# albtad01/NBody-EuroHPC

Hardware: AMD Instinct MI355X
Metric: body-interactions/s (higher is better)
Workload: dtype f32; 1 GPU; murb galaxy N=200000 steps=474 dt=3600 soft=2e8 seed=0 fp32 — BASELINE.json configs[2]: N=200000 i=200, 1 x MI355X; n_bodies=200000, parallelism=1 gpu, kernel_variant=8, jsplit=1, sym_waves=4, taper_pct=5, sym_passes=1

## Files before the change

include/murbhip.h:

```cpp
#ifndef MURBHIP_H_
#define MURBHIP_H_

#include <stddef.h>

#ifdef __cplusplus
extern "C" {
#endif

typedef struct murbhip_ctx murbhip_ctx;

#define MURBHIP_UNIQUE_ID_BYTES 128

#define MURBHIP_E_INVALID (-2000)
#define MURBHIP_E_STATE (-2001)
#define MURBHIP_E_NO_DEVICE (-2002)
#define MURBHIP_E_NO_RCCL (-2003)
#define MURBHIP_E_NOMEM (-2004)


int murbhip_version(void);

const char* murbhip_error_string(int code);

int murbhip_partition(unsigned long n, int world, int rank, unsigned long* first, unsigned long* count);

unsigned long murbhip_slice_slots(unsigned long n, int world);

unsigned long murbhip_slot_of_body(unsigned long n, int world, unsigned long i);

int murbhip_schedule_items(unsigned long n, int world, int rank, int split, int* pairs, unsigned long capacity,
                           unsigned long* count, unsigned long* own_count);

int murbhip_schedule_layout(unsigned long n, int world, int rank, int split, int waves, int taper_pct, int tri_first_pct,
                            int exchange_mode, long* items, unsigned long item_capacity, unsigned long* item_count, long* rows,
                            unsigned long row_capacity, unsigned long* row_count, unsigned long* floats_main,
                            unsigned long* floats_tri);


int murbhip_device_count(int* count);

int murbhip_create(murbhip_ctx** out, unsigned long n, float soft, float g, int device);

int murbhip_create_sharded(murbhip_ctx** out, unsigned long n, float soft, float g, int ndev, const int* devices,
                           int exchange);

int murbhip_unique_id(void* id_out );
int murbhip_create_rank(murbhip_ctx** out, unsigned long n, float soft, float g, int device, int rank, int world,
                        const void* unique_id);

int murbhip_destroy(murbhip_ctx* ctx);


int murbhip_upload(murbhip_ctx* ctx, const float* qx, const float* qy, const float* qz, const float* vx,
                   const float* vy, const float* vz, const float* m);

int murbhip_init_bodies(murbhip_ctx* ctx, const char* scheme, unsigned long seed);

int murbhip_download_mass(murbhip_ctx* ctx, float* m, float* r);

int murbhip_download_state(murbhip_ctx* ctx, float* qx, float* qy, float* qz, float* vx, float* vy, float* vz);

int murbhip_download_acc(murbhip_ctx* ctx, float* ax, float* ay, float* az);


int murbhip_compute_acc(murbhip_ctx* ctx);

int murbhip_compute_acc_jerk(murbhip_ctx* ctx);

int murbhip_download_jerk(murbhip_ctx* ctx, float* jx, float* jy, float* jz);
// ... 44 lines not shown
```

nbody-eurohpc_amd/csrc/murb_choose.h:

```cpp
#ifndef MURB_CHOOSE_H_
#define MURB_CHOOSE_H_

#include <algorithm>
#include <cstddef>

#include "murb_layout.h"
#include "murb_plan.h"

namespace {

struct PlanInputs {
    unsigned long n = 0;
    int world = 1;
    unsigned long slice = 0;
    unsigned long slots = 0;
    int cu_count = 0;
    size_t device_mem = 0;
    int resident_per_cu = 0;
    int variant = 0, jsplit = 0;
    int sym_waves = 0;
    int taper = -1;
    int diag_tri = -1;
    int sym_red = -1;
    int fuse_integrate = 1;
    long sym_pass_mb = 0;
    int tri_div = 0;
};

constexpr int kMaxParts = 64;
constexpr int kNumVariants = 8;
constexpr int kOneSidedVariant = 1;
constexpr int kOneSidedFewBodies = 2;
constexpr int kPersistentVariant = 7;
constexpr int kSymmetricVariant = 8;
constexpr unsigned long kSymmetricMinBodies = 2049;
constexpr int kRowsPerLaunch = kMaxParts / 2;

struct Plan {
    int variant;
    int parts_local, parts_remote;
    bool persistent;
    bool symmetric;
    int split;
    int waves;
    int taper;
    bool diag_tri;
    int red;
    MurbSchedule sched[2];
};

constexpr double kSymFastMaxReach = 0x1p34;
constexpr double kSymFastMinSoft = 0x1p-40;
inline bool sym_wide_needed(double reach, double soft) { return !(reach <= kSymFastMaxReach && soft >= kSymFastMinSoft); }
inline bool sym_wide_chosen(int option, bool needed) { return option < 0 ? needed : option != 0; }

inline int resident_blocks(const PlanInputs& in) { return std::max(in.resident_per_cu, 1) * std::max(in.cu_count, 1); }

inline MurbSchedule make_schedule(const PlanInputs& in, long groups, long tiles, int row_base)
{
    MurbSchedule sc{(int)groups, (int)tiles, 1, row_base};
    const long units = groups * tiles;
    if (units <= 0) { sc.nblocks = 0; return sc; }
    const long slots = resident_blocks(in);
    long rounds = in.jsplit > 0 ? in.jsplit : std::min<long>(8, std::max<long>(1, units / (slots * 8)));
    long nb = std::min(units, slots * rounds);
    nb = std::min(nb, std::max<long>(1, (kRowsPerLaunch - 2) * groups));
    sc.nblocks = (int)std::max<long>(nb, 1);
    return sc;
}

inline int variant_group(int variant)
{
    switch (variant) {
        case kPersistentVariant: return 32;
        case kSymmetricVariant: return 32;
        case 2: case 6: return 16;
        case 5: return 64;
        default: return 32;
    }
}
// ... 33 lines not shown
{
    const unsigned long T = in.slots / MURB_SYM_BLOCK;
    return in.fuse_integrate && in.jsplit == 0 && (T <= 4 || T == 6);
}

inline Plan make_plan(const PlanInputs& in)
{
    Plan p{};
    const auto fits = [&](int split) { return in.world == 1 || in.device_mem == 0 || sym_row_bytes(in, split) < in.device_mem / 2; };
    if (in.variant >= 1 && in.variant <= kNumVariants) p.variant = in.variant;
    else if (in.world == 1) p.variant = (in.n >= kSymmetricMinBodies && !fused_one_sided_wins(in) && fits(1)) ? kSymmetricVariant : kOneSidedVariant;
    else p.variant = (sym_items_per_rank(in) >= 400 && fits(1)) ? kSymmetricVariant : (in.slice <= 16384 ? kOneSidedFewBodies : kOneSidedVariant);
    p.symmetric = p.variant == kSymmetricVariant;
    if (p.symmetric) {
        const long items = sym_items_per_rank(in);
        const long want = (in.world > 1 ? 16L : 8L) * 4 * std::max(in.cu_count, 1);
        p.split = (in.jsplit == 1 || in.jsplit == 2 || in.jsplit == 4 || in.jsplit == 8 || in.jsplit == 16)
                      ? in.jsplit
                      : (items >= want ? 1 : (2 * items >= want ? 2 : (in.world == 1 || items >= 1000 ? 4 : (items >= 400 ? 8 : 16))));
        struct SmallPlan { int waves, split, taper; bool diag_tri; };
        static const SmallPlan kSmallPlans[5] = {{8, 4, 30, true}, {4, 4, 5, false}, {4, 8, 5, false}, {8, 8, 30, true}, {4, 16, 5, false}};
        static const signed char kSmallPlanOfBlocks[25] = {4, 4, 4, 3, 3, 3, 4,
                                                           3, 3, 0, 2, 2, 1, 3, 0, 2, 1, 2, 0, 1, 2, 0, 1, 0, 2};
        const int T = (int)(in.slots / MURB_SYM_BLOCK);
        const bool small = in.world == 1 && T <= 27;
        const SmallPlan sp = kSmallPlans[(small && in.cu_count == 256 && T >= 3) ? kSmallPlanOfBlocks[T - 3] : (T < 10 ? 3 : 0)];
        p.waves = (in.sym_waves == 4 || in.sym_waves == 8) ? in.sym_waves : (small ? sp.waves : 4);
        if (in.jsplit == 0 && in.sym_waves == 0 && small) p.split = sp.split;
        while (p.split > 1 && MURB_SYM_BLOCK / p.split < 16 * p.waves) p.split /= 2;
        while (p.split > 1 && !fits(p.split)) p.split /= 2;
        p.taper = in.taper >= 0 ? in.taper : (in.world > 1 ? 0 : (small ? sp.taper : (in.n <= 600000 ? 5 : 0)));
        p.diag_tri = in.diag_tri >= 0 ? in.diag_tri != 0 : (small && sp.diag_tri);
        p.red = in.sym_red >= 0 ? in.sym_red : 1;
        p.persistent = false;
        p.parts_local = p.parts_remote = 0;
        return p;
    }
    const unsigned long tiles_local = in.slice / MURB_TILE_BODIES;
    const unsigned long tiles_remote = (in.slots - in.slice) / MURB_TILE_BODIES;
    p.persistent = p.variant == kPersistentVariant;
    if (p.persistent) {
        unsigned long first, count;
        partition(in.n, in.world, 0, &first, &count);
        const long groups = (long)((count + 31) / 32);
        p.sched[0] = make_schedule(in, groups, (long)tiles_local, 0);
        p.sched[1] = make_schedule(in, groups, (long)tiles_remote, kRowsPerLaunch);
        p.parts_local = p.parts_remote = 0;
        return p;
    }
    if (in.world == 1) {
        p.parts_local = in.jsplit > 0 ? std::min<int>(in.jsplit, (int)std::min<unsigned long>(tiles_local, kMaxParts))
                                      : auto_parts(in, p.variant, in.slice, tiles_local);
        if (in.jsplit == 0 && in.fuse_integrate && p.variant == kOneSidedVariant && in.slots / MURB_SYM_BLOCK <= 6) p.parts_local = 1;
        p.parts_remote = 0;
    } else {
        const unsigned long tiles_all = tiles_local + tiles_remote;
        int total = in.jsplit > 0 ? in.jsplit : auto_parts(in, p.variant, in.slice, tiles_all);
        total = std::max(total, 2);
        int loc = (int)std::max<unsigned long>(1ul, (unsigned long)total * tiles_local / tiles_all);
        int rem = std::max(1, total - loc);
        p.parts_local = (int)std::min<unsigned long>((unsigned long)loc, std::min<unsigned long>(tiles_local, kMaxParts / 2));
        p.parts_remote = (int)std::min<unsigned long>((unsigned long)rem, std::min<unsigned long>(tiles_remote, kMaxParts / 2));
    }
    return p;
}

inline int plan_tri_div(const PlanInputs& in, const Plan& p)
{
    if (in.tri_div > 0) return in.tri_div;
    if (in.world == 1) return 1;
    const long tb = (long)(in.slice / MURB_SYM_BLOCK);
    const long items = tb * (tb + 1) / 2 * p.split / 2;
    const long slots = 4L * std::max(in.cu_count, 1) * 4 / p.waves;
    int div = 1;
    while (div < 4 && items * div < 2 * slots && MURB_SYM_BLOCK / (p.split * div * 2) >= 16 * p.waves) div *= 2;
    return div;
}

inline SymLayoutKey sym_layout_key(const PlanInputs& in, const Plan& p, bool exchange_mode, int overlap, int tri_first_pct, bool xcd_order,
                                   bool pad_aware)
{
    SymLayoutKey k;
    k.split = p.split; k.waves = p.waves; k.taper = p.taper; k.diag_tri = p.diag_tri;
    k.exchange_mode = exchange_mode;
    k.overlap = exchange_mode ? overlap : 0;
    k.tri_first_pct = exchange_mode ? tri_first_pct : 0;
    k.xcd_order = xcd_order;
    k.budget_floats = sym_pass_budget(in) / (3 * sizeof(float));
    k.tri_div = plan_tri_div(in, p);
    k.pad_aware = pad_aware;
    return k;
}

inline int hermite_parts(const PlanInputs& in)
{
    const unsigned long tiles = in.slots / MURB_TILE_BODIES;
    if (in.jsplit > 0) return (int)std::min<unsigned long>((unsigned long)in.jsplit, std::min<unsigned long>(tiles, kMaxParts / 2));
    return auto_parts(in, kOneSidedFewBodies, in.slots, tiles);
}

}

#endif
```

nbody-eurohpc_amd/csrc/murb_plan.h:

```cpp
#ifndef MURB_PLAN_H_
#define MURB_PLAN_H_

#include <cstddef>
#include <map>
#include <utility>
#include <vector>

#include "murb_schedule.h"
#include "murb_sym_types.h"

namespace {

struct SymPass {
    int item_first = 0, item_count = 0;
    int table_first = 0, table_count = 0;
    size_t floats = 0;
};

inline std::vector<std::pair<size_t, size_t>> cut_passes(const std::vector<SymPiece>& pieces, size_t budget_floats)
{
    std::vector<std::pair<size_t, size_t>> out;
    size_t first = 0, used = 0, k = 0;
    while (k < pieces.size()) {
        size_t e = k, rows = 0;
// ... 25 lines not shown
    for (size_t k = first; k < end; ++k) {
        const SymPiece& pc = pieces[k];
        const int bi = index[pc.i_slot0 / MURB_SYM_BLOCK];
        auto f = irow[bi].find(pc.J);
        if (f == irow[bi].end()) f = irow[bi].emplace(pc.J, table[bi].ni++).first;
        item_irow[k - first] = f->second;
        item_jrow[k - first] = pc.j_side() ? table[index[pc.J]].nj++ : -1;
    }
    size_t floats = 0;
    for (MurbSymBlockRows& br : table) {
        br.base_j = floats; floats += (size_t)br.nj * MURB_SYM_BLOCK;
        br.base_i = floats; floats += (size_t)br.ni * MURB_SYM_BLOCK;
    }
    for (size_t k = first; k < end; ++k) {
        const SymPiece& pc = pieces[k];
        MurbSymItem& it = items[k];
        it.i_slot0 = pc.i_slot0;
        it.ngroups = pc.len / (waves * MURB_SYM_R);
        it.J = pc.J;
        it.flags = pc.flags;
        const MurbSymBlockRows& bi = table[index[pc.i_slot0 / MURB_SYM_BLOCK]];
        it.ioff = bi.base_i + (size_t)item_irow[k - first] * MURB_SYM_BLOCK + (size_t)(pc.i_slot0 % MURB_SYM_BLOCK);
        it.joff = pc.j_side() ? table[index[pc.J]].base_j + (size_t)item_jrow[k - first] * MURB_SYM_BLOCK : 0;
    }
    return floats;
}

struct SymHostLayout {
    std::vector<MurbSymItem> items;
    int own = 0, t1 = 0;
    std::vector<MurbSymBlockRows> table_main, table_tri;
    size_t floats_main = 0, floats_tri = 0;
    std::vector<SymPass> passes;
};

struct SymLayoutKey {
    int split = 1, waves = 4, taper = 0;
    bool diag_tri = false;
    bool exchange_mode = false;
    int overlap = 0, tri_first_pct = 0;
    bool xcd_order = false;
    size_t budget_floats = 0;
    int tri_div = 1;
    bool pad_aware = true;
    bool operator==(const SymLayoutKey& o) const
    {
        return split == o.split && waves == o.waves && taper == o.taper && diag_tri == o.diag_tri && exchange_mode == o.exchange_mode &&
               overlap == o.overlap && tri_first_pct == o.tri_first_pct && xcd_order == o.xcd_order && budget_floats == o.budget_floats &&
               tri_div == o.tri_div && pad_aware == o.pad_aware;
    }
};

inline void plan_sym_layout(int W, int r, const SymFill& fill, const SymLayoutKey& key, SymHostLayout& L)
{
    const int tb = fill.tb;
    std::vector<int> flat;
    int own = 0;
    size_t t1 = 0;
    std::vector<SymPiece> pieces;
    std::vector<size_t> piece_ends;
    const auto build_pieces = [&](bool interleaved) {
        sym_schedule_items(W, r, tb, key.split, fill, flat, &own, interleaved);
        const size_t n_all = flat.size() / 2;
        t1 = (key.exchange_mode && key.overlap == 1) ? (size_t)((long)own * key.tri_first_pct / 100) : 0;
        std::vector<size_t> launch_ends;
        std::vector<int> launch_div;
        if (key.exchange_mode) {
            if (t1 > 0) { launch_ends.push_back(t1); launch_div.push_back(key.tri_div); }
            if ((size_t)own > t1) { launch_ends.push_back((size_t)own); launch_div.push_back(key.tri_div); }
            if (n_all > (size_t)own) { launch_ends.push_back(n_all); launch_div.push_back(1); }
        } else {
            launch_ends.push_back(n_all);
        }
        sym_pieces(flat, key.split, key.taper, 16 * key.waves, key.diag_tri, fill, launch_ends, pieces, piece_ends, launch_div);
    };
    build_pieces(key.xcd_order);
    if (!key.exchange_mode && key.xcd_order && cut_passes(pieces, key.budget_floats).size() > 1) build_pieces(false);
    size_t own_pieces = pieces.size();
    if (key.exchange_mode && flat.size() / 2 > (size_t)own) own_pieces = piece_ends.size() >= 2 ? piece_ends[piece_ends.size() - 2] : 0;
    L.items.assign(pieces.size(), MurbSymItem{});
    L.table_main.clear(); L.table_tri.clear();
    L.floats_main = L.floats_tri = 0;
    if (key.exchange_mode) {
        L.floats_tri = layout_sym_set(pieces, 0, own_pieces, key.waves, L.items, L.table_tri, [&](int b) { return std::make_pair(0, b - r * tb); });
        L.floats_main = layout_sym_set(pieces, own_pieces, pieces.size(), key.waves, L.items, L.table_main,
                                       [&](int b) { return std::make_pair(b / tb, b % tb); });
        L.passes.assign(1, SymPass{(int)own_pieces, (int)(pieces.size() - own_pieces), 0, (int)L.table_main.size(), L.floats_main});
    } else {
        L.passes.clear();
        std::vector<MurbSymBlockRows> table;
        for (const auto& range : cut_passes(pieces, key.budget_floats)) {
            const size_t floats = layout_sym_set(pieces, range.first, range.second, key.waves, L.items, table, [&](int b) { return std::make_pair(0, b); });
            L.passes.push_back(SymPass{(int)range.first, (int)(range.second - range.first), (int)L.table_main.size(), (int)table.size(), floats});
            L.table_main.insert(L.table_main.end(), table.begin(), table.end());
            L.floats_main = std::max(L.floats_main, floats);
        }
    }
    L.own = (int)own_pieces;
    L.t1 = t1 > 0 ? (int)piece_ends[0] : 0;
}

}

#endif
```

nbody-eurohpc_amd/csrc/murb_schedule.h:

```cpp
#ifndef MURB_SCHEDULE_H_
#define MURB_SCHEDULE_H_

#include <algorithm>
#include <vector>

#include "murb_layout.h"

namespace {

inline void partition(unsigned long n, int world, int rank, unsigned long* first, unsigned long* count)
{
    const unsigned long base = n / (unsigned long)world, rem = n % (unsigned long)world;
    const unsigned long r = (unsigned long)rank;
    *count = base + (r < rem ? 1 : 0);
    *first = r * base + std::min(r, rem);
}

inline unsigned long slice_slots(unsigned long n, int world)
{
    unsigned long first, count;
    partition(n, world, 0, &first, &count);
    return murb_round_up_tile(std::max(count, 1ul));
}

// ... 79 lines not shown
            const size_t row_first = flat.size();
            for (int j = 0; j < tb; ++j) {
                if (shared && !((r == lo) ? (a < hb) : (j >= hb))) continue;
                int ib, jb;
                sym_orient(fill, r * tb + a, s * tb + j, &ib, &jb);
                if (ib == r * tb + a) { flat.push_back(ib); flat.push_back(jb); }
                else sym_push_block_pair(fill, split, ib, jb, swapped);
            }
            const std::vector<int> row(flat.begin() + (long)row_first, flat.end());
            flat.resize(row_first);
            const int len = MURB_SLICE_ALIGN / split, real = fill.of(r * tb + a);
            for (int q = 0; q < split && q * len < real; ++q)
                for (size_t k = 0; k < row.size(); k += 2) { flat.push_back(row[k] * split + q); flat.push_back(row[k + 1]); }
        }
        flat.insert(flat.end(), swapped.begin(), swapped.end());
    }
    if (!xcd_order) return;
    const size_t n_own = (size_t)*own, n_all = flat.size() / 2;
    if (W == 1) { xcd_interleave(flat, 0, n_all); return; }
    xcd_interleave(flat, 0, n_own / 2);
    xcd_interleave(flat, n_own / 2, n_own);
    xcd_interleave(flat, n_own, n_all);
}

struct SymPiece {
    int i_slot0, len, J, flags;
    bool diag() const { return i_slot0 / MURB_SLICE_ALIGN == J; }
    bool j_side() const { return (flags & 1) == 0; }
};
constexpr int kSymStepBodies = 128;

inline void sym_pieces(const std::vector<int>& flat, int split, int taper_pct, int min_len, bool diag_tri, const SymFill& fill,
                       const std::vector<size_t>& launch_ends, std::vector<SymPiece>& out, std::vector<size_t>& piece_launch_ends,
                       const std::vector<int>& launch_div = std::vector<int>())
{
    const int len = MURB_SLICE_ALIGN / split;
    out.clear();
    piece_launch_ends.clear();
    size_t first = 0;
    for (size_t l = 0; l < launch_ends.size(); ++l) {
        const size_t end = launch_ends[l];
        const int base_div = l < launch_div.size() ? launch_div[l] : 1;
        const double total = (double)(end - first);
        for (size_t k = first; k < end; ++k) {
            const int isub = flat[2 * k], J = flat[2 * k + 1];
            const bool diag = isub / split == J;
            const double before = (double)(k - first) / (total > 0 ? total : 1.0);
            int div = 1;
            while (div < base_div && len / (2 * div) >= min_len) div *= 2;
            if (taper_pct > 0) {
                const double left = 1.0 - before;
                for (double f = taper_pct / 100.0; left <= f && len / (2 * div) >= min_len; f *= 0.5) div *= 2;
            }
            if (diag && diag_tri)
                while (len / div > kSymStepBodies && len / (2 * div) >= min_len) div *= 2;
            const int real_end = (isub / split) * MURB_SLICE_ALIGN + fill.of(isub / split);
            for (int q = 0; q < div; ++q) {
                SymPiece pc{isub * len + q * (len / div), len / div, J, diag ? 1 : 0};
                if (pc.i_slot0 >= real_end) break;
                if (pc.i_slot0 + pc.len > real_end) pc.len = (real_end - pc.i_slot0 + min_len - 1) / min_len * min_len;
                if (diag && diag_tri && pc.len <= kSymStepBodies) {
                    const int in_block = pc.i_slot0 % MURB_SLICE_ALIGN;
                    const int a = in_block / kSymStepBodies, b = (in_block + pc.len + kSymStepBodies - 1) / kSymStepBodies;
                    pc.flags = 2 | (a << 8) | (b << 12) | (b >= MURB_SLICE_ALIGN / kSymStepBodies ? 1 : 0);
                }
                out.push_back(pc);
            }
        }
        piece_launch_ends.push_back(out.size());
        first = end;
    }
}

}

#endif
```

nbody-eurohpc_amd/csrc/murbhip.hip:

```cpp
#include <hip/hip_runtime.h>

#include <algorithm>
#include <cmath>
#include <cstdio>
#include <cstdlib>
#include <cstring>
#include <functional>
#include <new>
#include <string>
#include <type_traits>
#include <vector>

#include "../../include/murbhip.h"
#include "murb_init.h"
#include "murb_ctx.h"

namespace {

constexpr int kPotentialKernel = 100;

inline bool is_idle(const murbhip_ctx* c, const Shard& sh) { return c->solo_shard >= 0 && sh.rank != c->solo_shard; }

template <int MODE, int R, int WAVES, int STAGE>
int launch_force_t(const MurbForceArgs& a, int i_slots, hipStream_t s)
// ... 1049 lines not shown
    partition(n, world, rank, first, count);
    return 0;
}

unsigned long murbhip_slice_slots(unsigned long n, int world) { return world < 1 ? 0 : slice_slots(n, world); }

unsigned long murbhip_slot_of_body(unsigned long n, int world, unsigned long i)
{
    if (world < 1 || i >= n) return ~0ul;
    const unsigned long base = n / (unsigned long)world, rem = n % (unsigned long)world;
    unsigned long r, first;
    if (i < rem * (base + 1)) { r = i / (base + 1); first = r * (base + 1); }
    else { r = rem + (base ? (i - rem * (base + 1)) / base : 0); first = rem * (base + 1) + (r - rem) * base; }
    return r * slice_slots(n, world) + (i - first);
}

int murbhip_schedule_items(unsigned long n, int world, int rank, int split, int* pairs, unsigned long capacity,
                           unsigned long* count, unsigned long* own_count)
{
    if (world < 1 || world > MURB_SYM_MAX_RANKS || rank < 0 || rank >= world || !count || !own_count) return MURBHIP_E_INVALID;
    if (split != 1 && split != 2 && split != 4 && split != 8 && split != 16) return MURBHIP_E_INVALID;
    std::vector<int> flat;
    int own = 0;
    sym_schedule_items(world, rank, (int)(slice_slots(n, world) / MURB_SYM_BLOCK), split, sym_fill(n, world), flat, &own);
    *count = flat.size() / 2;
    *own_count = (unsigned long)own;
    if (pairs) {
        if (capacity < flat.size() / 2) return MURBHIP_E_INVALID;
        std::memcpy(pairs, flat.data(), flat.size() * sizeof(int));
    }
    return 0;
}

int murbhip_schedule_layout(unsigned long n, int world, int rank, int split, int waves, int taper_pct, int tri_first_pct,
                            int exchange_mode, long* items, unsigned long item_capacity, unsigned long* item_count, long* rows,
                            unsigned long row_capacity, unsigned long* row_count, unsigned long* floats_main,
                            unsigned long* floats_tri)
{
    if (world < 1 || world > MURB_SYM_MAX_RANKS || rank < 0 || rank >= world || !item_count || !row_count) return MURBHIP_E_INVALID;
    if (split != 1 && split != 2 && split != 4 && split != 8 && split != 16) return MURBHIP_E_INVALID;
    if ((waves != 4 && waves != 8) || taper_pct < 0 || (taper_pct & 0xff) > 100 || taper_pct > 0x7ff || tri_first_pct < 0 || tri_first_pct > 100)
        return MURBHIP_E_INVALID;
    if (MURB_SYM_BLOCK / split < 16 * waves) return MURBHIP_E_INVALID;
    SymHostLayout L;
    SymLayoutKey key;
    key.split = split; key.waves = waves; key.taper = taper_pct & 0xff; key.diag_tri = (taper_pct & 0x100) != 0;
    key.exchange_mode = exchange_mode != 0 || world > 1;
    key.overlap = 1; key.tri_first_pct = tri_first_pct; key.tri_div = 1 << ((taper_pct >> 9) & 3);
    plan_sym_layout(world, rank, sym_fill(n, world), key, L);
    *item_count = L.items.size();
    *row_count = L.table_main.size() + L.table_tri.size();
    if (floats_main) *floats_main = L.floats_main;
    if (floats_tri) *floats_tri = L.floats_tri;
    if (items) {
        if (item_capacity < L.items.size()) return MURBHIP_E_INVALID;
        const bool ex = key.exchange_mode;
        for (size_t k = 0; k < L.items.size(); ++k) {
            const MurbSymItem& it = L.items[k];
            long* o = items + 8 * k;
            o[0] = it.i_slot0; o[1] = (long)it.ngroups * waves * MURB_SYM_R; o[2] = it.J; o[3] = it.flags;
            o[4] = (ex && (int)k < L.own) ? 1 : 0;
            o[5] = (long)it.ioff; o[6] = (long)it.joff;
            o[7] = !ex ? 0 : ((int)k < L.t1 ? 0 : ((int)k < L.own ? 1 : 2));
        }
    }
    if (rows) {
        if (row_capacity < *row_count) return MURBHIP_E_INVALID;
        size_t e = 0;
        for (int set = 0; set < 2; ++set)
            for (const MurbSymBlockRows& br : (set == 0 ? L.table_main : L.table_tri)) {
                long* o = rows + 7 * e++;
                o[0] = set; o[1] = br.out_slice; o[2] = br.out_block; o[3] = (long)br.base_i; o[4] = br.ni; o[5] = (long)br.base_j; o[6] = br.nj;
            }
    }
    return 0;
}

int murbhip_device_count(int* count)
{
    if (!count) return MURBHIP_E_INVALID;
    *count = 0;
    return hip_rc(hipGetDeviceCount(count));
}

int murbhip_create(murbhip_ctx** out, unsigned long n, float soft, float g, int device)
{
    const int rank0 = 0;
    return create_common(out, n, soft, g, 1, 1, &device, &rank0, 0, false);
}

int murbhip_create_sharded(murbhip_ctx** out, unsigned long n, float soft, float g, int ndev, const int* devices,
                           int exchange)
{
    if (ndev < 1 || ndev > 64 || !devices || (exchange != 0 && exchange != 1)) return MURBHIP_E_INVALID;
    if ((unsigned long)ndev > n) return MURBHIP_E_INVALID;
    std::vector<int> ranks(ndev);
    for (int i = 0; i < ndev; ++i) ranks[i] = i;
    if (exchange == 1) {
        if (!rccl().ok) return MURBHIP_E_NO_RCCL;
    }
    RC_TRY(create_common(out, n, soft, g, ndev, ndev, devices, ranks.data(), exchange, false));
    if (exchange == 1 && ndev > 1) {
        std::vector<rccl_comm_t> comms(ndev);
        const int rc = nccl_rc(rccl().CommInitAll(comms.data(), ndev, devices));
        if (rc != 0) { murbhip_destroy(*out); *out = nullptr; return rc; }
        for (int i = 0; i < ndev; ++i) (*out)->shards[i].comm_rccl = comms[i];
    }
    return 0;
// ... 761 lines not shown
    double sums[MURB_METRIC_VALUES];
    RC_TRY(device_metrics(c, false, sums));
    std::memcpy(out10, sums + 2, 10 * sizeof(double));
    return 0;
}

int murbhip_set_option(murbhip_ctx* c, const char* key, long value)
{
    if (!c || !key) return MURBHIP_E_INVALID;
    const std::string k(key);
    if (k == "solo_shard" || k == "force_exchange") c->acc_current = false;
    if (k == "variant") { if (value < 0 || value > kNumVariants) return MURBHIP_E_INVALID; c->in.variant = (int)value; }
    else if (k == "jsplit") { if (value < 0 || value > kMaxParts / 2) return MURBHIP_E_INVALID; c->in.jsplit = (int)value; }
    else if (k == "xcd_order") c->xcd_order = value ? 1 : 0;
    else if (k == "pad_aware") c->pad_aware = value ? 1 : 0;
    else if (k == "energy_sweep") c->energy_sweep = value ? 1 : 0;
    else if (k == "sym_wide") {
        if (value < -1 || value > 1) return MURBHIP_E_INVALID;
        if ((int)value != c->sym_wide) { c->acc_current = false; c->pe_current = false; }
        c->sym_wide = (int)value;
    }
    else if (k == "fuse_integrate") c->in.fuse_integrate = value ? 1 : 0;
    else if (k == "exchange_p2p") {
        if (value && (c->exchange != 1 || !rccl().Send || !rccl().Recv)) return MURBHIP_E_STATE;
        RC_TRY(murbhip_sync(c));
        c->exchange_p2p = value ? 1 : 0;
    }
    else if (k == "tri_div") { if (value != 0 && value != 1 && value != 2 && value != 4 && value != 8) return MURBHIP_E_INVALID; c->in.tri_div = (int)value; }
    else if (k == "init_libm_fma") { if (value < -1 || value > 1) return MURBHIP_E_INVALID; c->init_libm_fma = (int)value; }
    else if (k == "tri_first_pct") { if (value < 0 || value > 100) return MURBHIP_E_INVALID; c->tri_first_pct = (int)value; }
    else if (k == "taper") { if (value < -1 || value > 100) return MURBHIP_E_INVALID; c->in.taper = (int)value; }
    else if (k == "sym_pass_mb") { if (value < 0) return MURBHIP_E_INVALID; c->in.sym_pass_mb = value; }
    else if (k == "diag_tri") { if (value < -1 || value > 1) return MURBHIP_E_INVALID; c->in.diag_tri = (int)value; }
    else if (k == "sym_red") { if (value < -1 || value > 1) return MURBHIP_E_INVALID; c->in.sym_red = (int)value; }
    else if (k == "sym_waves") { if (value != 0 && value != 4 && value != 8) return MURBHIP_E_INVALID; c->in.sym_waves = (int)value; }
    else if (k == "overlap") { if (value < 0 || value > 2) return MURBHIP_E_INVALID; c->overlap = (int)value; }
    else if (k == "integrator") {
        if (value < 0 || value > 2) return MURBHIP_E_INVALID;
        if (c->lf_half && value != c->integrator) return MURBHIP_E_STATE;
        if (value == 2 && (c->in.world != 1 || c->shards.size() != 1 || c->force_exchange)) return MURBHIP_E_STATE;
        if (value != 2 && (c->nearest || c->contact)) return MURBHIP_E_STATE;
        c->integrator = (int)value;
    }
    else if (k == "evolve_batch") {
        if (value < 0 || value > kEvolveBatch) return MURBHIP_E_INVALID;
        c->evolve_batch = (int)value;
    }
    else if (k == "nearest") {
        if (value != 0 && value != 1) return MURBHIP_E_INVALID;
        if (c->integrator != 2 || c->in.world != 1 || c->shards.size() != 1) return MURBHIP_E_STATE;
        if (value && c->contact) return MURBHIP_E_STATE;
        if (!value && c->enc_radius > 0.f) return MURBHIP_E_STATE;
        if ((int)value != c->nearest) {
            c->nearest = (int)value;
            invalidate_cached_forces(c);
        }
    }
    else if (k == "contact") {
        if (value < 0 || value > 2) return MURBHIP_E_INVALID;
        if (c->integrator != 2 || c->in.world != 1 || c->shards.size() != 1) return MURBHIP_E_STATE;
        if (value && c->nearest) return MURBHIP_E_STATE;
        const bool was = c->contact != 0, now = value != 0;
        if (was != now) {
            if (c->blk_open) return MURBHIP_E_STATE;
            c->contact = (int)value;
            c->enc_count = 0;
// ... 43 lines not shown
    return 0;
}

int murbhip_get_info(murbhip_ctx* c, const char* key, double* value)
{
    if (!c || !key || !value) return MURBHIP_E_INVALID;
    const std::string k(key);
    const Plan p = current_plan(c);
    if (k == "cu_count") *value = c->in.cu_count;
    else if (k == "clock_mhz") *value = c->clock_mhz;
    else if (k == "n") *value = (double)c->in.n;
    else if (k == "slots") *value = (double)c->in.slots;
    else if (k == "world") *value = c->in.world;
    else if (k == "cu_reserve") *value = c->cu_reserve;
    else if (k == "sym_passes") *value = c->shards[0].sym_main.passes.empty() ? 0.0 : (double)c->shards[0].sym_main.passes.size();
    else if (k == "rank") *value = c->shards[0].rank;
    else if (k == "jsplit") *value = p.symmetric ? (double)p.split
                                     : p.persistent ? (double)p.sched[0].nblocks / std::max(resident_blocks(c->in), 1)
                                                    : (double)(p.parts_local + p.parts_remote);
    else if (k == "hermite_parts") *value = hermite_parts(c->in);
    else if (k == "block_units") *value = block_units(c);
    else if (k == "block_grid") *value = block_grid(c);
    else if (k == "nearest") *value = c->nearest;
    else if (k == "encounter_count") *value = c->contact ? 0.0 : (double)c->enc_count;
    else if (k == "contact") *value = c->contact;
    else if (k == "contact_count") *value = c->contact ? (double)c->enc_count : 0.0;
    else if (k == "block_steps") *value = c->blk_info[0];
    else if (k == "block_body_steps") *value = c->blk_info[1];
    else if (k == "block_clamped") *value = c->blk_info[2];
    else if (k == "block_max_active") *value = c->blk_info[3];
    else if (k == "sym_waves") *value = p.symmetric ? p.waves : 0;
    else if (k == "sym_wide") *value = p.symmetric && sym_wide_chosen(c->sym_wide, c->sym_wide_needed) ? 1 : 0;
    else if (k == "taper") *value = p.symmetric ? p.taper : 0;
    else if (k == "workgroups") *value = p.persistent ? p.sched[0].nblocks + (c->in.world > 1 ? p.sched[1].nblocks : 0) : 0;
    else if (k == "variant") *value = p.variant;
    else if (k == "interactions_per_launch") *value = c->interactions_per_launch;
    else if (k == "device_bytes") { double b = 0; for (Shard& sh : c->shards) b += (double)sh.bytes; *value = b; }
    else if (k == "sym_launches") { double v = 0; for (Shard& sh : c->shards) v += (double)sh.sym_launches; *value = v; }
    else if (k == "spans_dropped") {
        *value = 0;
        for (Shard& sh : c->shards) if (!sh.prof.empty() && sh.prof_used + 2 > sh.prof.size()) *value = 1;
    }
    else if (k == "force_launches" || k == "force_ms_avg" || k == "force_ms_total" || k.rfind("span_", 0) == 0 || k == "compute_wait_ms_per_step") {
        static const char* const names[kProfKinds] = {"force", "tri1", "rect", "tri2", "reduce_scatter", "all_gather", "wait_gather",
                                                      "wait_reduce", "step"};
        RC_TRY(murbhip_sync(c));
        double total[kProfKinds] = {0};
        size_t count[kProfKinds] = {0};
        for (Shard& sh : c->shards) {
            HIP_TRY(hipSetDevice(sh.device));
            for (size_t i = 0; i + 1 < sh.prof_used; i += 2) {
                float ms = 0.f;
                HIP_TRY(hipEventElapsedTime(&ms, sh.prof[i], sh.prof[i + 1]));
                const int kind = sh.prof_kind[i / 2];
                total[kind] += ms; ++count[kind];
            }
        }
        const double f_total = total[kProfForce] + total[kProfTri1] + total[kProfRect] + total[kProfTri2];
        const size_t f_count = count[kProfForce] + count[kProfTri1] + count[kProfRect] + count[kProfTri2];
        if (k == "force_launches") *value = (double)f_count;
        else if (k == "force_ms_total") *value = f_total;
        else if (k == "force_ms_avg") *value = f_count ? f_total / (double)f_count : 0.0;
        else if (k == "compute_wait_ms_per_step")
            *value = count[kProfStep] ? (total[kProfWaitGather] + total[kProfWaitReduce]) / (double)count[kProfStep] : 0.0;
        else {
            const bool avg = k.size() > 7 && k.compare(k.size() - 7, 7, "_ms_avg") == 0;
// ... 14 lines not shown
```

nbody-eurohpc_amd/murbhip/__init__.py:

```python
import ctypes as C
import os

import numpy as np

_HERE = os.path.dirname(os.path.abspath(__file__))
LIB_PATH = os.environ.get("MURBHIP_LIBRARY") or os.path.join(_HERE, "..", "lib", "libmurbhip.so")
G = np.float32(6.67384e-11)

_fp = C.POINTER(C.c_float)


class MurbHipError(RuntimeError):
    def __init__(self, code, what):
        self.code = code
        super().__init__(f"{what}: {error_string(code)} (code {code})")


_lib = None


def lib():
    global _lib
    if _lib is None:
        path = os.path.normpath(LIB_PATH)
        if not os.path.exists(path):
            raise FileNotFoundError(f"{path} is missing: build it with `make -C nbody-eurohpc_amd` "
                                    "(there is no CPU fallback for the HIP path)")
        L = C.CDLL(path)
        L.murbhip_version.restype = C.c_int
        L.murbhip_error_string.restype = C.c_char_p
        L.murbhip_error_string.argtypes = [C.c_int]
        L.murbhip_partition.argtypes = [C.c_ulong, C.c_int, C.c_int, C.POINTER(C.c_ulong), C.POINTER(C.c_ulong)]
        L.murbhip_slice_slots.restype = C.c_ulong
        L.murbhip_slice_slots.argtypes = [C.c_ulong, C.c_int]
        L.murbhip_slot_of_body.restype = C.c_ulong
        L.murbhip_slot_of_body.argtypes = [C.c_ulong, C.c_int, C.c_ulong]
        L.murbhip_schedule_items.argtypes = [C.c_ulong, C.c_int, C.c_int, C.c_int, C.POINTER(C.c_int), C.c_ulong,
                                             C.POINTER(C.c_ulong), C.POINTER(C.c_ulong)]
        L.murbhip_schedule_layout.argtypes = [C.c_ulong] + [C.c_int] * 7 + [C.POINTER(C.c_long), C.c_ulong, C.POINTER(C.c_ulong),
                                                                            C.POINTER(C.c_long), C.c_ulong, C.POINTER(C.c_ulong),
                                                                            C.POINTER(C.c_ulong), C.POINTER(C.c_ulong)]
        L.murbhip_device_count.argtypes = [C.POINTER(C.c_int)]
        L.murbhip_create.argtypes = [C.POINTER(C.c_void_p), C.c_ulong, C.c_float, C.c_float, C.c_int]
        L.murbhip_create_sharded.argtypes = [C.POINTER(C.c_void_p), C.c_ulong, C.c_float, C.c_float, C.c_int,
                                             C.POINTER(C.c_int), C.c_int]
        L.murbhip_unique_id.argtypes = [C.c_void_p]
        L.murbhip_create_rank.argtypes = [C.POINTER(C.c_void_p), C.c_ulong, C.c_float, C.c_float, C.c_int, C.c_int,
                                          C.c_int, C.c_void_p]
        L.murbhip_destroy.argtypes = [C.c_void_p]
        L.murbhip_upload.argtypes = [C.c_void_p] + [_fp] * 7
        L.murbhip_init_bodies.argtypes = [C.c_void_p, C.c_char_p, C.c_ulong]
        L.murbhip_download_mass.argtypes = [C.c_void_p, _fp, _fp]
        L.murbhip_download_state.argtypes = [C.c_void_p] + [_fp] * 6
        L.murbhip_download_acc.argtypes = [C.c_void_p] + [_fp] * 3
        L.murbhip_compute_acc.argtypes = [C.c_void_p]
        L.murbhip_compute_acc_jerk.argtypes = [C.c_void_p]
        L.murbhip_download_jerk.argtypes = [C.c_void_p] + [_fp] * 3
        L.murbhip_evolve.argtypes = [C.c_void_p, C.c_double, C.c_double, C.c_double, C.c_float, C.c_float, C.c_ulong,
                                     C.POINTER(C.c_double)]
        L.murbhip_evolve_dts.argtypes = [C.c_void_p, _fp, C.c_ulong, C.POINTER(C.c_ulong)]
        L.murbhip_evolve_block.argtypes = [C.c_void_p, C.c_float, C.c_ulong, C.c_double, C.c_double, C.c_int, C.c_ulong,
                                           C.POINTER(C.c_double)]
        L.murbhip_block_state.argtypes = [C.c_void_p, C.POINTER(C.c_uint), C.POINTER(C.c_int)]
        L.murbhip_block_set_levels.argtypes = [C.c_void_p, C.POINTER(C.c_int), C.c_int]
        L.murbhip_download_nearest.argtypes = [C.c_void_p, C.POINTER(C.c_int), _fp]
        L.murbhip_set_encounter.argtypes = [C.c_void_p, C.c_float]
        L.murbhip_encounters.argtypes = [C.c_void_p, C.POINTER(C.c_int), C.POINTER(C.c_int), _fp, C.c_ulong, C.POINTER(C.c_ulong),
                                         C.POINTER(C.c_double)]
        L.murbhip_upload_radii.argtypes = [C.c_void_p, _fp]
        L.murbhip_download_contact.argtypes = [C.c_void_p, C.POINTER(C.c_int), _fp]
        L.murbhip_contacts.argtypes = [C.c_void_p, C.POINTER(C.c_int), C.POINTER(C.c_int), _fp, C.c_ulong, C.POINTER(C.c_ulong),
                                       C.POINTER(C.c_double)]
        L.murbhip_warmup.argtypes = [C.c_void_p, C.c_double]
        L.murbhip_step.argtypes = [C.c_void_p, C.c_float]
        L.murbhip_steps.argtypes = [C.c_void_p, C.c_float, C.c_int]
        L.murbhip_integrate_host_acc.argtypes = [C.c_void_p] + [_fp] * 3 + [C.c_float]
        L.murbhip_sync.argtypes = [C.c_void_p]
        L.murbhip_energy.argtypes = [C.c_void_p, C.POINTER(C.c_double), C.POINTER(C.c_double)]
        L.murbhip_moments.argtypes = [C.c_void_p, C.POINTER(C.c_double)]
        L.murbhip_set_option.argtypes = [C.c_void_p, C.c_char_p, C.c_long]
        L.murbhip_get_info.argtypes = [C.c_void_p, C.c_char_p, C.POINTER(C.c_double)]
        _lib = L
    return _lib


EXPORTS = ("murbhip_version murbhip_error_string murbhip_partition murbhip_slice_slots murbhip_slot_of_body "
           "murbhip_schedule_items murbhip_schedule_layout "
           "murbhip_device_count murbhip_create murbhip_create_sharded murbhip_unique_id murbhip_create_rank "
           "murbhip_destroy murbhip_upload murbhip_init_bodies murbhip_download_mass murbhip_download_state murbhip_download_acc murbhip_compute_acc "
           "murbhip_compute_acc_jerk murbhip_download_jerk murbhip_evolve murbhip_evolve_dts "
           "murbhip_evolve_block murbhip_block_state murbhip_block_set_levels "
           "murbhip_download_nearest murbhip_set_encounter murbhip_encounters "
           "murbhip_upload_radii murbhip_download_contact murbhip_contacts "
           "murbhip_warmup murbhip_step murbhip_steps murbhip_integrate_host_acc murbhip_sync murbhip_energy murbhip_moments murbhip_set_option "
           "murbhip_get_info").split()


def error_string(code):
    return lib().murbhip_error_string(code).decode()


def _check(code, what):
    if code != 0:
        raise MurbHipError(code, what)


def _ptr(a):
    return a.ctypes.data_as(_fp)


def _f32(a):
    return np.ascontiguousarray(a, dtype=np.float32)


def partition(n, world, rank):
    first, count = C.c_ulong(), C.c_ulong()
    _check(lib().murbhip_partition(n, world, rank, C.byref(first), C.byref(count)), "murbhip_partition")
    return first.value, count.value


def slice_slots(n, world):
    return lib().murbhip_slice_slots(n, world)


def slot_of_body(n, world, i):
    return lib().murbhip_slot_of_body(n, world, i)


def schedule_items(n, world, rank, split=1):
    count, own = C.c_ulong(), C.c_ulong()
    _check(lib().murbhip_schedule_items(n, world, rank, split, None, 0, C.byref(count), C.byref(own)),
           "murbhip_schedule_items")
    items = np.zeros((count.value, 2), np.int32)
    _check(lib().murbhip_schedule_items(n, world, rank, split, items.ctypes.data_as(C.POINTER(C.c_int)), count.value,
                                        C.byref(count), C.byref(own)), "murbhip_schedule_items")
    return items, own.value


def schedule_layout(n, world, rank, split=1, waves=4, taper=0, tri_first_pct=50, exchange_mode=False, diag_tri=False, tri_div=1):
    ni, nr, fm, ft = C.c_ulong(), C.c_ulong(), C.c_ulong(), C.c_ulong()
    args = (n, world, rank, split, waves, taper + (256 if diag_tri else 0) + 512 * {1: 0, 2: 1, 4: 2, 8: 3}[tri_div], tri_first_pct,
            int(exchange_mode))
    _check(lib().murbhip_schedule_layout(*args, None, 0, C.byref(ni), None, 0, C.byref(nr), C.byref(fm), C.byref(ft)),
           "murbhip_schedule_layout")
    items = np.zeros((ni.value, 8), np.int64)
    rows = np.zeros((nr.value, 7), np.int64)
    lp = C.POINTER(C.c_long)
    _check(lib().murbhip_schedule_layout(*args, items.ctypes.data_as(lp), ni.value, C.byref(ni), rows.ctypes.data_as(lp), nr.value,
                                         C.byref(nr), C.byref(fm), C.byref(ft)), "murbhip_schedule_layout")
    return items, rows, fm.value, ft.value


def device_count():
    c = C.c_int(0)
    rc = lib().murbhip_device_count(C.byref(c))
    return c.value if rc == 0 else 0


def unique_id():
    buf = C.create_string_buffer(128)
    _check(lib().murbhip_unique_id(buf), "murbhip_unique_id")
    return buf.raw


class Simulation:

    def __init__(self, n, soft=2e8, g=G, device=0, devices=None, exchange="copy", rank=None, world=None, uid=None):
        self.n = int(n)
        self._h = C.c_void_p()
        L = lib()
        if devices is not None:
            arr = (C.c_int * len(devices))(*devices)
            _check(L.murbhip_create_sharded(C.byref(self._h), self.n, soft, g, len(devices), arr,
                                            {"copy": 0, "rccl": 1}[exchange]), "murbhip_create_sharded")
        elif rank is not None:
            _check(L.murbhip_create_rank(C.byref(self._h), self.n, soft, g, device, rank, world, uid),
                   "murbhip_create_rank")
        else:
            _check(L.murbhip_create(C.byref(self._h), self.n, soft, g, device), "murbhip_create")

    def upload(self, s):
        a = [_f32(s[k]) for k in ("qx", "qy", "qz", "vx", "vy", "vz", "m")]
        for x in a:
# ... 391 lines not shown
```

Measured before the change: 6294 billion interactions/s.

## Move diagonal tile work to a fine-grained tail at end of each launch

Adds a diag_tail option to the symmetric schedule. For single-GPU runs with at least 45000 bodies, the diagonal (self-block) items are pulled out of the tapered ordering and appended at the end of each launch as small pieces of 16*waves rows. This aims to fill the end-of-launch drain with fine-grained work and reduce load imbalance. The tail is dropped if it would force a multi-pass layout. Items now vary more in size and the schedule gains extra host logic.

```diff
diff --git a/include/murbhip.h b/include/murbhip.h
--- a/include/murbhip.h
+++ b/include/murbhip.h
@@ -35,6 +35,11 @@
                             int exchange_mode, long* items, unsigned long item_capacity, unsigned long* item_count, long* rows,
                             unsigned long row_capacity, unsigned long* row_count, unsigned long* floats_main,
                             unsigned long* floats_tri);
+
+int murbhip_schedule_layout_tail(unsigned long n, int world, int rank, int split, int waves, int taper_pct, int tri_first_pct,
+                                 int exchange_mode, int diag_tail, int* diag_tail_used, long* items, unsigned long item_capacity,
+                                 unsigned long* item_count, long* rows, unsigned long row_capacity, unsigned long* row_count,
+                                 unsigned long* floats_main, unsigned long* floats_tri);
 
 
 int murbhip_device_count(int* count);
diff --git a/nbody-eurohpc_amd/csrc/murb_choose.h b/nbody-eurohpc_amd/csrc/murb_choose.h
--- a/nbody-eurohpc_amd/csrc/murb_choose.h
+++ b/nbody-eurohpc_amd/csrc/murb_choose.h
@@ -25,6 +25,7 @@
     int fuse_integrate = 1;
     long sym_pass_mb = 0;
     int tri_div = 0;
+    int diag_tail = -1;
 };
 
 constexpr int kMaxParts = 64;
@@ -35,6 +36,7 @@
 constexpr int kSymmetricVariant = 8;
 constexpr unsigned long kSymmetricMinBodies = 2049;
 constexpr int kRowsPerLaunch = kMaxParts / 2;
+constexpr unsigned long kDiagTailMinBodies = 45000;
 
 struct Plan {
     int variant;
@@ -46,6 +48,7 @@
     int taper;
     bool diag_tri;
     int red;
+    int diag_tail;
     MurbSchedule sched[2];
 };
 
@@ -145,6 +148,7 @@
         p.taper = in.taper >= 0 ? in.taper : (in.world > 1 ? 0 : (small ? sp.taper : (in.n <= 600000 ? 5 : 0)));
         p.diag_tri = in.diag_tri >= 0 ? in.diag_tri != 0 : (small && sp.diag_tri);
         p.red = in.sym_red >= 0 ? in.sym_red : 1;
+        p.diag_tail = in.diag_tail >= 0 ? in.diag_tail : (in.world == 1 && in.n >= kDiagTailMinBodies && !p.diag_tri ? 16 * p.waves : 0);
         p.persistent = false;
         p.parts_local = p.parts_remote = 0;
         return p;
@@ -190,6 +194,26 @@
     return div;
 }
 
+inline bool diag_tail_valid(long value, int waves) { return value == -1 || (value >= 0 && value <= MURB_SYM_BLOCK && value % (16 * waves) == 0); }
+
+inline bool sym_single_pass(const PlanInputs& in, const Plan& p)
+{
+    const size_t budget = sym_pass_budget(in) / (3 * sizeof(float));
+    if (budget == 0) return true;
+    const double tb = (double)(in.slots / MURB_SYM_BLOCK), pairs = tb * (tb + 1) / 2, off = tb * (tb - 1) / 2 * p.split;
+    int levels = 0;
+    for (int len = MURB_SYM_BLOCK / p.split; len / 2 >= 16 * p.waves; len /= 2) ++levels;
+    const double rows = pairs + off + levels * (p.taper / 100.0) * pairs * p.split + (double)(1 << levels) + 1;
+    return rows * MURB_SYM_BLOCK <= (double)budget;
+}
+
+inline int plan_diag_tail(const PlanInputs& in, const Plan& p, bool exchange_mode, bool xcd_order)
+{
+    if (!p.symmetric || in.world > 1 || exchange_mode || xcd_order || p.diag_tri) return 0;
+    if (p.diag_tail <= 0 || !diag_tail_valid(p.diag_tail, p.waves)) return 0;
+    return sym_single_pass(in, p) ? p.diag_tail : 0;
+}
+
 inline SymLayoutKey sym_layout_key(const PlanInputs& in, const Plan& p, bool exchange_mode, int overlap, int tri_first_pct, bool xcd_order,
                                    bool pad_aware)
 {
@@ -202,6 +226,7 @@
     k.budget_floats = sym_pass_budget(in) / (3 * sizeof(float));
     k.tri_div = plan_tri_div(in, p);
     k.pad_aware = pad_aware;
+    k.diag_tail = plan_diag_tail(in, p, exchange_mode, xcd_order);
     return k;
 }
 
diff --git a/nbody-eurohpc_amd/csrc/murb_plan.h b/nbody-eurohpc_amd/csrc/murb_plan.h
--- a/nbody-eurohpc_amd/csrc/murb_plan.h
+++ b/nbody-eurohpc_amd/csrc/murb_plan.h
@@ -81,6 +81,7 @@
     std::vector<MurbSymBlockRows> table_main, table_tri;
     size_t floats_main = 0, floats_tri = 0;
     std::vector<SymPass> passes;
+    int diag_tail = 0;
 };
 
 struct SymLayoutKey {
@@ -92,13 +93,21 @@
     size_t budget_floats = 0;
     int tri_div = 1;
     bool pad_aware = true;
+    int diag_tail = 0;
     bool operator==(const SymLayoutKey& o) const
     {
         return split == o.split && waves == o.waves && taper == o.taper && diag_tri == o.diag_tri && exchange_mode == o.exchange_mode &&
                overlap == o.overlap && tri_first_pct == o.tri_first_pct && xcd_order == o.xcd_order && budget_floats == o.budget_floats &&
-               tri_div == o.tri_div && pad_aware == o.pad_aware;
+               tri_div == o.tri_div && pad_aware == o.pad_aware && diag_tail == o.diag_tail;
     }
 };
+
+inline int sym_diag_tail_usable(int W, const SymLayoutKey& key)
+{
+    const bool ok = W == 1 && !key.exchange_mode && !key.diag_tri && !key.xcd_order && key.diag_tail > 0 &&
+                    key.diag_tail % (16 * key.waves) == 0 && key.diag_tail <= MURB_SYM_BLOCK;
+    return ok ? key.diag_tail : 0;
+}
 
 inline void plan_sym_layout(int W, int r, const SymFill& fill, const SymLayoutKey& key, SymHostLayout& L)
 {
@@ -108,6 +117,7 @@
     size_t t1 = 0;
     std::vector<SymPiece> pieces;
     std::vector<size_t> piece_ends;
+    int diag_tail = sym_diag_tail_usable(W, key);
     const auto build_pieces = [&](bool interleaved) {
         sym_schedule_items(W, r, tb, key.split, fill, flat, &own, interleaved);
         const size_t n_all = flat.size() / 2;
@@ -121,10 +131,12 @@
         } else {
             launch_ends.push_back(n_all);
         }
-        sym_pieces(flat, key.split, key.taper, 16 * key.waves, key.diag_tri, fill, launch_ends, pieces, piece_ends, launch_div);
+        sym_pieces(flat, key.split, key.taper, 16 * key.waves, key.diag_tri, fill, launch_ends, pieces, piece_ends, launch_div, diag_tail);
     };
     build_pieces(key.xcd_order);
     if (!key.exchange_mode && key.xcd_order && cut_passes(pieces, key.budget_floats).size() > 1) build_pieces(false);
+    if (diag_tail > 0 && cut_passes(pieces, key.budget_floats).size() > 1) { diag_tail = 0; build_pieces(false); }
+    L.diag_tail = diag_tail;
     size_t own_pieces = pieces.size();
     if (key.exchange_mode && flat.size() / 2 > (size_t)own) own_pieces = piece_ends.size() >= 2 ? piece_ends[piece_ends.size() - 2] : 0;
     L.items.assign(pieces.size(), MurbSymItem{});
diff --git a/nbody-eurohpc_amd/csrc/murb_schedule.h b/nbody-eurohpc_amd/csrc/murb_schedule.h
--- a/nbody-eurohpc_amd/csrc/murb_schedule.h
+++ b/nbody-eurohpc_amd/csrc/murb_schedule.h
@@ -135,7 +135,7 @@
 
 inline void sym_pieces(const std::vector<int>& flat, int split, int taper_pct, int min_len, bool diag_tri, const SymFill& fill,
                        const std::vector<size_t>& launch_ends, std::vector<SymPiece>& out, std::vector<size_t>& piece_launch_ends,
-                       const std::vector<int>& launch_div = std::vector<int>())
+                       const std::vector<int>& launch_div = std::vector<int>(), int diag_tail = 0)
 {
     const int len = MURB_SLICE_ALIGN / split;
     out.clear();
@@ -145,10 +145,12 @@
         const size_t end = launch_ends[l];
         const int base_div = l < launch_div.size() ? launch_div[l] : 1;
         const double total = (double)(end - first);
+        size_t tailed = 0;
         for (size_t k = first; k < end; ++k) {
             const int isub = flat[2 * k], J = flat[2 * k + 1];
             const bool diag = isub / split == J;
-            const double before = (double)(k - first) / (total > 0 ? total : 1.0);
+            if (diag && diag_tail > 0) { ++tailed; continue; }
+            const double before = (double)(k - first - tailed) / (total > 0 ? total : 1.0);
             int div = 1;
             while (div < base_div && len / (2 * div) >= min_len) div *= 2;
             if (taper_pct > 0) {
@@ -170,6 +172,16 @@
                 out.push_back(pc);
             }
         }
+        for (size_t k = first; tailed > 0 && k < end; ++k) {
+            const int isub = flat[2 * k], J = flat[2 * k + 1];
+            if (isub / split != J) continue;
+            const int item_end = (isub + 1) * len, real_end = J * MURB_SLICE_ALIGN + fill.of(J);
+            for (int s = isub * len; s < item_end && s < real_end; s += diag_tail) {
+                SymPiece pc{s, std::min(diag_tail, item_end - s), J, 1};
+                if (pc.i_slot0 + pc.len > real_end) pc.len = (real_end - pc.i_slot0 + min_len - 1) / min_len * min_len;
+                out.push_back(pc);
+            }
+        }
         piece_launch_ends.push_back(out.size());
         first = end;
     }
diff --git a/nbody-eurohpc_amd/csrc/murbhip.hip b/nbody-eurohpc_amd/csrc/murbhip.hip
--- a/nbody-eurohpc_amd/csrc/murbhip.hip
+++ b/nbody-eurohpc_amd/csrc/murbhip.hip
@@ -1105,22 +1105,24 @@
     return 0;
 }
 
-int murbhip_schedule_layout(unsigned long n, int world, int rank, int split, int waves, int taper_pct, int tri_first_pct,
-                            int exchange_mode, long* items, unsigned long item_capacity, unsigned long* item_count, long* rows,
-                            unsigned long row_capacity, unsigned long* row_count, unsigned long* floats_main,
-                            unsigned long* floats_tri)
+int murbhip_schedule_layout_tail(unsigned long n, int world, int rank, int split, int waves, int taper_pct, int tri_first_pct,
+                                 int exchange_mode, int diag_tail, int* diag_tail_used, long* items, unsigned long item_capacity,
+                                 unsigned long* item_count, long* rows, unsigned long row_capacity, unsigned long* row_count,
+                                 unsigned long* floats_main, unsigned long* floats_tri)
 {
     if (world < 1 || world > MURB_SYM_MAX_RANKS || rank < 0 || rank >= world || !item_count || !row_count) return MURBHIP_E_INVALID;
     if (split != 1 && split != 2 && split != 4 && split != 8 && split != 16) return MURBHIP_E_INVALID;
     if ((waves != 4 && waves != 8) || taper_pct < 0 || (taper_pct & 0xff) > 100 || taper_pct > 0x7ff || tri_first_pct < 0 || tri_first_pct > 100)
         return MURBHIP_E_INVALID;
-    if (MURB_SYM_BLOCK / split < 16 * waves) return MURBHIP_E_INVALID;
+    if (MURB_SYM_BLOCK / split < 16 * waves || diag_tail < 0 || !diag_tail_valid(diag_tail, waves)) return MURBHIP_E_INVALID;
     SymHostLayout L;
     SymLayoutKey key;
     key.split = split; key.waves = waves; key.taper = taper_pct & 0xff; key.diag_tri = (taper_pct & 0x100) != 0;
     key.exchange_mode = exchange_mode != 0 || world > 1;
     key.overlap = 1; key.tri_first_pct = tri_first_pct; key.tri_div = 1 << ((taper_pct >> 9) & 3);
+    key.diag_tail = diag_tail;
     plan_sym_layout(world, rank, sym_fill(n, world), key, L);
+    if (diag_tail_used) *diag_tail_used = L.diag_tail;
     *item_count = L.items.size();
     *row_count = L.table_main.size() + L.table_tri.size();
     if (floats_main) *floats_main = L.floats_main;
@@ -1147,6 +1149,15 @@
             }
     }
     return 0;
+}
+
+int murbhip_schedule_layout(unsigned long n, int world, int rank, int split, int waves, int taper_pct, int tri_first_pct,
+                            int exchange_mode, long* items, unsigned long item_capacity, unsigned long* item_count, long* rows,
+                            unsigned long row_capacity, unsigned long* row_count, unsigned long* floats_main,
+                            unsigned long* floats_tri)
+{
+    return murbhip_schedule_layout_tail(n, world, rank, split, waves, taper_pct, tri_first_pct, exchange_mode, 0, nullptr, items, item_capacity,
+                                        item_count, rows, row_capacity, row_count, floats_main, floats_tri);
 }
 
 int murbhip_device_count(int* count)
@@ -1974,6 +1985,12 @@
     else if (k == "taper") { if (value < -1 || value > 100) return MURBHIP_E_INVALID; c->in.taper = (int)value; }
     else if (k == "sym_pass_mb") { if (value < 0) return MURBHIP_E_INVALID; c->in.sym_pass_mb = value; }
     else if (k == "diag_tri") { if (value < -1 || value > 1) return MURBHIP_E_INVALID; c->in.diag_tri = (int)value; }
+    else if (k == "diag_tail") {
+        const Plan p = current_plan(c);
+        if (!diag_tail_valid(value, p.symmetric ? p.waves : 4)) return MURBHIP_E_INVALID;
+        if ((int)value != c->in.diag_tail) { c->acc_current = false; c->pe_current = false; }
+        c->in.diag_tail = (int)value;
+    }
     else if (k == "sym_red") { if (value < -1 || value > 1) return MURBHIP_E_INVALID; c->in.sym_red = (int)value; }
     else if (k == "sym_waves") { if (value != 0 && value != 4 && value != 8) return MURBHIP_E_INVALID; c->in.sym_waves = (int)value; }
     else if (k == "overlap") { if (value < 0 || value > 2) return MURBHIP_E_INVALID; c->overlap = (int)value; }
@@ -2083,6 +2100,7 @@
     else if (k == "sym_waves") *value = p.symmetric ? p.waves : 0;
     else if (k == "sym_wide") *value = p.symmetric && sym_wide_chosen(c->sym_wide, c->sym_wide_needed) ? 1 : 0;
     else if (k == "taper") *value = p.symmetric ? p.taper : 0;
+    else if (k == "diag_tail") *value = plan_diag_tail(c->in, p, exchange_mode(c), c->xcd_order != 0);
     else if (k == "workgroups") *value = p.persistent ? p.sched[0].nblocks + (c->in.world > 1 ? p.sched[1].nblocks : 0) : 0;
     else if (k == "variant") *value = p.variant;
     else if (k == "interactions_per_launch") *value = c->interactions_per_launch;
diff --git a/nbody-eurohpc_amd/murbhip/__init__.py b/nbody-eurohpc_amd/murbhip/__init__.py
--- a/nbody-eurohpc_amd/murbhip/__init__.py
+++ b/nbody-eurohpc_amd/murbhip/__init__.py
@@ -40,6 +40,7 @@
         L.murbhip_schedule_layout.argtypes = [C.c_ulong] + [C.c_int] * 7 + [C.POINTER(C.c_long), C.c_ulong, C.POINTER(C.c_ulong),
                                                                             C.POINTER(C.c_long), C.c_ulong, C.POINTER(C.c_ulong),
                                                                             C.POINTER(C.c_ulong), C.POINTER(C.c_ulong)]
+        L.murbhip_schedule_layout_tail.argtypes = [C.c_ulong] + [C.c_int] * 8 + [C.POINTER(C.c_int)] + L.murbhip_schedule_layout.argtypes[8:]
         L.murbhip_device_count.argtypes = [C.POINTER(C.c_int)]
         L.murbhip_create.argtypes = [C.POINTER(C.c_void_p), C.c_ulong, C.c_float, C.c_float, C.c_int]
         L.murbhip_create_sharded.argtypes = [C.POINTER(C.c_void_p), C.c_ulong, C.c_float, C.c_float, C.c_int,
@@ -85,7 +86,7 @@
 
 
 EXPORTS = ("murbhip_version murbhip_error_string murbhip_partition murbhip_slice_slots murbhip_slot_of_body "
-           "murbhip_schedule_items murbhip_schedule_layout "
+           "murbhip_schedule_items murbhip_schedule_layout murbhip_schedule_layout_tail "
            "murbhip_device_count murbhip_create murbhip_create_sharded murbhip_unique_id murbhip_create_rank "
            "murbhip_destroy murbhip_upload murbhip_init_bodies murbhip_download_mass murbhip_download_state murbhip_download_acc murbhip_compute_acc "
            "murbhip_compute_acc_jerk murbhip_download_jerk murbhip_evolve murbhip_evolve_dts "
@@ -137,18 +138,22 @@
     return items, own.value
 
 
-def schedule_layout(n, world, rank, split=1, waves=4, taper=0, tri_first_pct=50, exchange_mode=False, diag_tri=False, tri_div=1):
-    ni, nr, fm, ft = C.c_ulong(), C.c_ulong(), C.c_ulong(), C.c_ulong()
+def schedule_layout(n, world, rank, split=1, waves=4, taper=0, tri_first_pct=50, exchange_mode=False, diag_tri=False, tri_div=1,
+                    diag_tail=None):
+    ni, nr, fm, ft, used = C.c_ulong(), C.c_ulong(), C.c_ulong(), C.c_ulong(), C.c_int(0)
     args = (n, world, rank, split, waves, taper + (256 if diag_tri else 0) + 512 * {1: 0, 2: 1, 4: 2, 8: 3}[tri_div], tri_first_pct,
             int(exchange_mode))
-    _check(lib().murbhip_schedule_layout(*args, None, 0, C.byref(ni), None, 0, C.byref(nr), C.byref(fm), C.byref(ft)),
-           "murbhip_schedule_layout")
+    query, what = lib().murbhip_schedule_layout, "murbhip_schedule_layout"
+    if diag_tail is not None:
+        args += (diag_tail, C.byref(used))
+        query, what = lib().murbhip_schedule_layout_tail, "murbhip_schedule_layout_tail"
+    _check(query(*args, None, 0, C.byref(ni), None, 0, C.byref(nr), C.byref(fm), C.byref(ft)), what)
     items = np.zeros((ni.value, 8), np.int64)
     rows = np.zeros((nr.value, 7), np.int64)
     lp = C.POINTER(C.c_long)
-    _check(lib().murbhip_schedule_layout(*args, items.ctypes.data_as(lp), ni.value, C.byref(ni), rows.ctypes.data_as(lp), nr.value,
-                                         C.byref(nr), C.byref(fm), C.byref(ft)), "murbhip_schedule_layout")
-    return items, rows, fm.value, ft.value
+    _check(query(*args, items.ctypes.data_as(lp), ni.value, C.byref(ni), rows.ctypes.data_as(lp), nr.value, C.byref(nr), C.byref(fm),
+                 C.byref(ft)), what)
+    return (items, rows, fm.value, ft.value) + (() if diag_tail is None else (used.value,))
 
 
 def device_count():
```

After: 6320 billion interactions/s, median of 2. No clear change (+0.4%).
